# MobilePerceptionLab/EventCalib

Measured on NVIDIA B200. Metric: events/sec (detection+residual eval), higher is better.
Workload: dtype int32 pixels / f64 fit + f64 residuals

## Files before the change

eventcalib_b200/csrc/ecb_api.cu:

```cuda
#include <sched.h>
#include <math.h>
#include <stdarg.h>
#include <stdio.h>
#include <string.h>

#include <algorithm>

#include "ecb_window.cuh"

int ecb_fail(ecb_ctx *ctx, int code, const char *fmt, ...) {
    char buf[512];
    va_list ap;
    va_start(ap, fmt);
    vsnprintf(buf, sizeof buf, fmt, ap);
    va_end(ap);
    if (ctx) ctx->err = buf;
    return code;
}

int ecb_check(ecb_ctx *ctx, cudaError_t e, const char *what) {
    if (e == cudaSuccess) return ECB_OK;
    return ecb_fail(ctx, ECB_ERR_CUDA, "CUDA error %s: %s", what, cudaGetErrorString(e));
}

// ... 282 lines not shown

    if ((rc = ecb_reserve(ctx, ctx->win_t, (size_t) n_win * 16))) return rc;
    if ((rc = ecb_reserve(ctx, ctx->win_lohi, (size_t) n_win * 16))) return rc;
    if ((rc = ecb_reserve(ctx, ctx->win_ptoff, (size_t) n_win * 8))) return rc;
    if ((rc = ecb_h2d(ctx, ctx->win_t.p, windows, (size_t) n_win * 16))) return rc;
    if ((rc = ecb_launch_bounds(ctx, (const double *) ctx->win_t.p, n_win, (int64_t *) ctx->win_lohi.p))) return rc;
    ctx->h_lohi.resize((size_t) 2 * n_win);
    ctx->h_ptoff.resize((size_t) n_win);
    if ((rc = ecb_d2h(ctx, ctx->h_lohi.data(), ctx->win_lohi.p, (size_t) n_win * 16))) return rc;
    int64_t total = 0, max_cnt = 0;
    for (int w = 0; w < n_win; ++w) {
        int64_t cnt = std::max<int64_t>(0, ctx->h_lohi[2 * w + 1] - ctx->h_lohi[2 * w]);
        ctx->h_ptoff[w] = total;
        total += cnt;
        max_cnt = std::max(max_cnt, cnt);
    }
    if (max_cnt > 0x3FFFFFFF) return ecb_fail(ctx, ECB_ERR_UNSUPPORTED, "window with %lld events", (long long) max_cnt);
    ctx->total_points = total;
    if ((rc = ecb_h2d(ctx, ctx->win_ptoff.p, ctx->h_ptoff.data(), (size_t) n_win * 8))) return rc;

    const size_t slots = (size_t) std::max<int64_t>(total, 1);
    if ((rc = ecb_reserve(ctx, ctx->arrive, 2 * slots * 4))) return rc;
    for (int p = 0; p < 2; ++p) {
        if ((rc = ecb_reserve(ctx, ctx->pts[p], slots * 4))) return rc;
        if ((rc = ecb_reserve(ctx, ctx->labels[p], slots * 4))) return rc;
    }
    if ((rc = ecb_reserve(ctx, ctx->kmem, 2 * slots * 4))) return rc;
    if ((rc = ecb_reserve(ctx, ctx->db_dims, (size_t) 2 * n_win * sizeof(ProbDesc)))) return rc;
    if ((rc = ecb_reserve(ctx, ctx->db_hdr, (size_t) 2 * n_win * sizeof(ProbHdr)))) return rc;
    if ((rc = ecb_reserve(ctx, ctx->summary, (size_t) n_win * sizeof(ecb_window_summary)))) return rc;
    if ((rc = ecb_reserve(ctx, ctx->status, 64))) return rc;

    WindowArgs wa;
    wa.xyp = (const uint32_t *) ctx->ev_xyp.p;
    wa.lohi = (const int64_t *) ctx->win_lohi.p;
    wa.ptoff = (const int64_t *) ctx->win_ptoff.p;
    wa.arrive[0] = (uint32_t *) ctx->arrive.p;
    wa.arrive[1] = (uint32_t *) ctx->arrive.p + slots;
    wa.pts[0] = (uint32_t *) ctx->pts[0].p;
    wa.pts[1] = (uint32_t *) ctx->pts[1].p;
    wa.prob = (ProbDesc *) ctx->db_dims.p;
    wa.n_win = n_win;
    wa.W = ctx->width;
    wa.H = ctx->height;
    wa.max_n = (uint32_t *) ctx->status.p + 4;
    wa.order_mode = params->order_mode;
    ECB_CUDA(ctx, cudaMemsetAsync(ctx->status.p, 0, 64, ctx->stream));
    if ((rc = ecb_launch_window(ctx, wa))) return rc;
    uint32_t max_nm[2] = {0, 0};
    if ((rc = ecb_d2h(ctx, max_nm, wa.max_n, 8))) return rc;
    const uint32_t max_n = max_nm[0];
    if (params->order_mode == 1) {
        OrderArgs oa;
        memset(&oa, 0, sizeof oa);
        oa.prob = (const ProbDesc *) ctx->db_dims.p;
        oa.n_prob = 2 * n_win;
        oa.work_counter = (unsigned *) ctx->status.p;
        for (int p = 0; p < 2; ++p) {
            oa.arrive[p] = wa.arrive[p];
            oa.pts[p] = wa.pts[p];
        }
        if ((rc = ecb_launch_order(ctx, oa, (int) max_nm[1]))) return rc;
    }

  for (int attempt = 0;; ++attempt) {
    if ((rc = ecb_reserve(ctx, ctx->ktab, (size_t) 2 * n_win * max_k * sizeof(KeptCluster)))) return rc;
    ctx->cand_stride = max_k;
    if ((rc = ecb_reserve(ctx, ctx->cand, (size_t) n_win * ctx->cand_stride * 5 * 8))) return rc;
    uint32_t *const d_max_kept = (uint32_t *) ctx->status.p + 12;
    ca.max_kept = d_max_kept;
    ca.prob = (const ProbDesc *) ctx->db_dims.p;
    ca.n_prob = 2 * n_win;
    ca.work_counter = (unsigned *) ctx->status.p;
    for (int p = 0; p < 2; ++p) {
        ca.pix[p] = (const uint32_t *) ctx->pts[p].p;
        ca.labels[p] = (int32_t *) ctx->labels[p].p;
        ca.kmem[p] = (uint32_t *) ctx->kmem.p + p * slots;
    }
    ca.hdr = (ProbHdr *) ctx->db_hdr.p;
    ca.ktab = (KeptCluster *) ctx->ktab.p;
    ca.max_k = max_k;
    ca.W = ctx->width;
    ca.H = ctx->height;
    ca.PW = ((ca.W + 2 * ca.E + 31) >> 5) + 1;
    ca.PH = ca.H + 2 * ca.E;
    ca.min_pts = params->dbscan_min_pts;
    ca.cluster_min = params->cluster_min;
    const bool exact = params->median_mode == 1;
    int bfs_cap = 0;
    if (exact) {
        bfs_cap = (int) std::min<size_t>((size_t) 2 * n_win * max_k, 2 * slots / std::max<uint32_t>(params->cluster_min, 1u) + 16);
        if ((rc = ecb_reserve(ctx, ctx->kd_tree, 8 * slots * 4))) return rc;
        if ((rc = ecb_reserve(ctx, ctx->bfs_key, 2 * slots * 8))) return rc;
        if ((rc = ecb_reserve(ctx, ctx->bfs_items, (size_t) bfs_cap * sizeof(BfsItem) + 16))) return rc;
        ca.exact_order = 1;
        for (int p = 0; p < 2; ++p) ca.kd_nodes[p] = (uint32_t *) ctx->kd_tree.p + (size_t) (4 * p) * slots;
        ca.bfs_items = (BfsItem *) ((char *) ctx->bfs_items.p + 16);
        ca.bfs_count = (unsigned *) ctx->bfs_items.p;
        ca.bfs_cap = bfs_cap;
        ECB_CUDA(ctx, cudaMemsetAsync(ctx->bfs_items.p, 0, 16, ctx->stream));
    }
    if ((rc = ecb_launch_cluster(ctx, ca, (int) max_n))) return rc;
    if (exact) {
        BfsArgs ba;
        memset(&ba, 0, sizeof ba);
        ba.items = ca.bfs_items;
        ba.count = ca.bfs_count;
        ba.max_items = bfs_cap;
        ba.prob = ca.prob;
        for (int p = 0; p < 2; ++p) {
            ba.pix[p] = ca.pix[p];
            ba.labels[p] = ca.labels[p];
            ba.kd_nodes[p] = (const uint4 *) ca.kd_nodes[p];
            ba.members[p] = ca.kmem[p];
            ba.scratch[p] = wa.arrive[p];
            ba.key[p] = (unsigned long long *) ctx->bfs_key.p + (size_t) p * slots;
        }
        ba.init_keys = 1;
        ba.ktab = ca.ktab;
        ba.max_k = max_k;
        ba.eps = params->dbscan_eps;
        if ((rc = ecb_launch_bfs(ctx, ba))) return rc;
    }

    PairArgs pa;
    pa.prob = ca.prob;
    pa.hdr = ca.hdr;
    pa.ktab = ca.ktab;
    for (int p = 0; p < 2; ++p) {
        pa.pts[p] = ca.pix[p];
        pa.kmem[p] = ca.kmem[p];
    }
    pa.lohi = wa.lohi;
    pa.summary = (ecb_window_summary *) ctx->summary.p;
    pa.cand = (double *) ctx->cand.p;
    pa.n_win = n_win;
    pa.max_k = max_k;
    pa.cand_stride = ctx->cand_stride;
    pa.smem_cap = (int) max_n;
    pa.fit_circle = params->fit_circle;
    pa.knn_num = params->knn_num < 1 ? 1 : params->knn_num;
    pa.rows_cols = params->rows_cols;
    pa.rthr = params->radius_threshold;
    {
        static const int pair_dyn = getenv("ECB_PAIR_DYN") ? atoi(getenv("ECB_PAIR_DYN")) : 1;
        pa.win_counter = pair_dyn ? (unsigned *) ctx->status.p + 8 : nullptr;
    }
    if ((rc = ecb_launch_pair(ctx, pa))) return rc;
    if (!auto_k) break;
    uint32_t max_kept = 0;
    if ((rc = ecb_d2h(ctx, &max_kept, d_max_kept, 4))) return rc;
    if (max_kept <= (uint32_t) max_k) break;
    if (attempt >= 2) return ecb_fail(ctx, ECB_ERR_STATE, "kept-cluster table still too small after resizing (%u > %d)", max_kept, max_k);
    max_k = (int) ((max_kept + 63u) & ~63u);
    ctx->max_k_auto = max_k;
    ECB_CUDA(ctx, cudaMemsetAsync((uint32_t *) ctx->status.p + 8, 0, 32, ctx->stream));
  }
    ctx->n_win = n_win;
    return ECB_OK;
}

int ecb_frontend_summary(ecb_ctx *ctx, ecb_window_summary *out, int n_win) {
    if (!ctx || !out) return ECB_ERR_ARG;
    if (n_win > ctx->n_win) n_win = ctx->n_win;
    cudaSetDevice(ctx->device);
    return ecb_d2h(ctx, out, ctx->summary.p, (size_t) n_win * sizeof(ecb_window_summary));
}
// ... 122 lines not shown
}

int ecb_frontend_device_ptrs(ecb_ctx *ctx, void **d_summary, void **d_candidates, int *cand_stride) {
    if (!ctx) return ECB_ERR_ARG;
    if (d_summary) *d_summary = ctx->summary.p;
    if (d_candidates) *d_candidates = ctx->cand.p;
    if (cand_stride) *cand_stride = ctx->cand_stride;
    return ECB_OK;
}

static int dbscan_batch(ecb_ctx *ctx, const double *xy, const int64_t *offsets, int n_problems, double eps,
                        uint32_t min_pts, int32_t *labels, int32_t *n_clusters, uint32_t *status, int32_t *cluster_sizes,
                        uint32_t *members) {
    if (!ctx || !offsets || n_problems < 0 || (!xy && n_problems > 0)) return ECB_ERR_ARG;
    const bool ordered = cluster_sizes && members;
    if (min_pts < 1) return ecb_fail(ctx, ECB_FAILED, "min < 1 (dbscan.h:123)");
    cudaSetDevice(ctx->device);
    int rc;
    ClusterArgs ca;
    memset(&ca, 0, sizeof ca);
    if (n_problems == 0) return ECB_OK;
    auto general = [&]() {
        if (status)
            for (int k = 0; k < n_problems; ++k) status[k] = 0;
        return ecb_dbscan_general(ctx, xy, 2, offsets, n_problems, eps, min_pts, labels, n_clusters, cluster_sizes, members);
    };
    if (!(eps >= 1.0) || eps > ECB_MAX_EPS) return general();
    if ((rc = fill_stencil(ctx, ca, eps))) return rc;
    const int64_t total = offsets[n_problems];
    std::vector<uint32_t> pix((size_t) std::max<int64_t>(total, 1));
    std::vector<ProbDesc> pd((size_t) n_problems);
    int Wmax = 1, Hmax = 1, max_n = 0;
    for (int k = 0; k < n_problems; ++k) {
        const int64_t b = offsets[k], e = offsets[k + 1];
        if (e - b < 1) return ecb_fail(ctx, ECB_FAILED, "problem %d: V->size() < 1 (dbscan.h:121)", k);
        if (e - b > 0x3FFFFFFF) return ecb_fail(ctx, ECB_ERR_UNSUPPORTED, "problem %d too large", k);
        int xmin = 1 << 30, ymin = 1 << 30, xmax = -1, ymax = -1;
        for (int64_t i = b; i < e; ++i) {
            const double x = xy[2 * i], y = xy[2 * i + 1];
            const int xi = (int) x, yi = (int) y;
            if (!(x >= 0.0 && x < 32768.0 && y >= 0.0 && y < 32768.0 && (double) xi == x && (double) yi == y)) return general();
            pix[(size_t) i] = (uint32_t) xi | ((uint32_t) yi << 15);
            xmin = std::min(xmin, xi);
            ymin = std::min(ymin, yi);
            xmax = std::max(xmax, xi);
            ymax = std::max(ymax, yi);
        }
        ProbDesc d;
        memset(&d, 0, sizeof d);
        d.off = b;
        d.n = (int32_t) (e - b);
        d.pol = 0;
        d.x0 = xmin;
        d.y0 = ymin;
        pd[(size_t) k] = d;
        Wmax = std::max(Wmax, xmax - xmin + 1);
        Hmax = std::max(Hmax, ymax - ymin + 1);
        max_n = std::max(max_n, d.n);
    }
    if ((int64_t) (Wmax + 2 * ca.E + 64) * (Hmax + 2 * ca.E) > (1ll << 21)) return general();
    const size_t slots = (size_t) std::max<int64_t>(total, 1);
    const int max_k = 1;
    if ((rc = ecb_reserve(ctx, ctx->db_pix, slots * 4))) return rc;
    if ((rc = ecb_reserve(ctx, ctx->db_labels, slots * 4))) return rc;
    if ((rc = ecb_reserve(ctx, ctx->db_scratch, slots * 4))) return rc;
    if ((rc = ecb_reserve(ctx, ctx->db_off, (size_t) n_problems * sizeof(ProbDesc)))) return rc;
    if ((rc = ecb_reserve(ctx, ctx->db_hdr_b, (size_t) n_problems * sizeof(ProbHdr)))) return rc;
    if ((rc = ecb_reserve(ctx, ctx->db_ktab, (size_t) n_problems * max_k * sizeof(KeptCluster)))) return rc;
    if ((rc = ecb_reserve(ctx, ctx->db_counter, 64))) return rc;
    ECB_CUDA(ctx, cudaMemcpyAsync(ctx->db_pix.p, pix.data(), slots * 4, cudaMemcpyHostToDevice, ctx->stream));
    ECB_CUDA(ctx, cudaMemcpyAsync(ctx->db_off.p, pd.data(), (size_t) n_problems * sizeof(ProbDesc), cudaMemcpyHostToDevice,
                                  ctx->stream));
    ca.prob = (const ProbDesc *) ctx->db_off.p;
    ca.n_prob = n_problems;
    ca.work_counter = (unsigned *) ctx->db_counter.p;
    ca.pix[0] = ca.pix[1] = (const uint32_t *) ctx->db_pix.p;
    ca.labels[0] = ca.labels[1] = (int32_t *) ctx->db_labels.p;
    ca.kmem[0] = ca.kmem[1] = (uint32_t *) ctx->db_scratch.p;
    ca.hdr = (ProbHdr *) ctx->db_hdr_b.p;
    ca.ktab = (KeptCluster *) ctx->db_ktab.p;
    ca.max_k = max_k;
    ca.W = Wmax;
    ca.H = Hmax;
    ca.PW = ((ca.W + 2 * ca.E + 31) >> 5) + 1;
    ca.PH = ca.H + 2 * ca.E;
    ca.min_pts = min_pts;
    ca.cluster_min = 0x7FFFFFFF;
    ca.max_kept = nullptr;
    if (ordered) {
        if ((rc = ecb_reserve(ctx, ctx->kd_tree, 4 * slots * 4))) return rc;
        ca.exact_order = 1;
        ca.kd_nodes[0] = ca.kd_nodes[1] = (uint32_t *) ctx->kd_tree.p;
        ca.bfs_count = (unsigned *) ctx->db_counter.p + 4;
        ca.bfs_cap = 0;
    }
    if ((rc = ecb_launch_cluster(ctx, ca, max_n))) return rc;
    if (ordered) {
        if ((rc = ecb_reserve(ctx, ctx->bfs_key, slots * 8))) return rc;
        if ((rc = ecb_reserve(ctx, ctx->bfs_items, slots * sizeof(BfsItem) + 16))) return rc;
        if ((rc = ecb_reserve(ctx, ctx->bfs_front, slots * 4))) return rc;
        if ((rc = ecb_reserve(ctx, ctx->bfs_tab, 3 * slots * 4))) return rc;
        ECB_CUDA(ctx, cudaMemsetAsync(ctx->bfs_key.p, 0xFF, slots * 8, ctx->stream));
        ECB_CUDA(ctx, cudaMemsetAsync(ctx->bfs_items.p, 0, 16, ctx->stream));
        uint32_t *csize = (uint32_t *) ctx->bfs_tab.p, *cseed = csize + slots, *coff = cseed + slots;
        BfsItem *items = (BfsItem *) ((char *) ctx->bfs_items.p + 16);
        if ((rc = ecb_launch_bfs_all_items(ctx, ca.prob, ca.hdr, n_problems, ca.labels[0], csize, cseed, coff, items,
                                           (unsigned *) ctx->bfs_items.p, (int) slots)))
            return rc;
        BfsArgs ba;
        memset(&ba, 0, sizeof ba);
        ba.items = items;
        ba.count = (const unsigned *) ctx->bfs_items.p;
        ba.max_items = (int) slots;
        ba.prob = ca.prob;
        for (int p = 0; p < 2; ++p) {
            ba.pix[p] = ca.pix[0];
            ba.labels[p] = ca.labels[0];
            ba.kd_nodes[p] = (const uint4 *) ca.kd_nodes[0];
            ba.members[p] = (uint32_t *) ctx->db_scratch.p;
            ba.scratch[p] = (uint32_t *) ctx->bfs_front.p;
            ba.key[p] = (unsigned long long *) ctx->bfs_key.p;
        }
        ba.init_keys = 0;
        ba.eps = eps;
        if ((rc = ecb_launch_bfs(ctx, ba))) return rc;
        ECB_CUDA(ctx, cudaMemcpyAsync(members, ctx->db_scratch.p, (size_t) total * 4, cudaMemcpyDeviceToHost, ctx->stream));
        ECB_CUDA(ctx, cudaMemcpyAsync(cluster_sizes, csize, (size_t) total * 4, cudaMemcpyDeviceToHost, ctx->stream));
    }
    std::vector<ProbHdr> hdr((size_t) n_problems);
    if (labels) ECB_CUDA(ctx, cudaMemcpyAsync(labels, ctx->db_labels.p, (size_t) total * 4, cudaMemcpyDeviceToHost, ctx->stream));
    ECB_CUDA(ctx, cudaMemcpyAsync(hdr.data(), ctx->db_hdr_b.p, (size_t) n_problems * sizeof(ProbHdr), cudaMemcpyDeviceToHost,
                                  ctx->stream));
    ECB_CUDA(ctx, ecb_stream_sync(ctx));
    for (int k = 0; k < n_problems; ++k) {
        if (n_clusters) n_clusters[k] = hdr[(size_t) k].n_clusters;
        if (status) status[k] = hdr[(size_t) k].status;
        if (hdr[(size_t) k].status & ECB_PB_DUPLICATE) return general();
    }
    return ECB_OK;
}

int ecb_dbscan_run_batch(ecb_ctx *ctx, const double *xy, const int64_t *offsets, int n_problems, double eps,
                         uint32_t min_pts, int32_t *labels, int32_t *n_clusters, uint32_t *status) {
    return dbscan_batch(ctx, xy, offsets, n_problems, eps, min_pts, labels, n_clusters, status, nullptr, nullptr);
}

int ecb_dbscan_run_batch_ordered(ecb_ctx *ctx, const double *xy, const int64_t *offsets, int n_problems, double eps,
                                 uint32_t min_pts, int32_t *labels, int32_t *n_clusters, uint32_t *status,
                                 int32_t *cluster_sizes, uint32_t *members) {
    if (!cluster_sizes || !members) return ECB_ERR_ARG;
    return dbscan_batch(ctx, xy, offsets, n_problems, eps, min_pts, labels, n_clusters, status, cluster_sizes, members);
}

int ecb_dbscan_run_ordered(ecb_ctx *ctx, const double *xy, int n, double eps, uint32_t min_pts, int32_t *labels,
                           int32_t *n_clusters, int32_t *cluster_sizes, uint32_t *members) {
    if (!ctx || !cluster_sizes || !members) return ECB_ERR_ARG;
    if (n < 1 || min_pts < 1) return ECB_FAILED;
    const int64_t off[2] = {0, n};
    return dbscan_batch(ctx, xy, off, 1, eps, min_pts, labels, n_clusters, nullptr, cluster_sizes, members);
}

int ecb_dbscan_run_nd(ecb_ctx *ctx, const double *pts, int n, int dim, double eps, uint32_t min_pts, int32_t *labels,
                      int32_t *n_clusters, int32_t *cluster_sizes, uint32_t *members) {
    if (!ctx || (!pts && n > 0) || ((cluster_sizes == nullptr) != (members == nullptr))) return ECB_ERR_ARG;
    if (n < 1 || dim < 1 || min_pts < 1) return ECB_FAILED;
    const int64_t off[2] = {0, n};
    if (dim == 2) return dbscan_batch(ctx, pts, off, 1, eps, min_pts, labels, n_clusters, nullptr, cluster_sizes, members);
// ... 85 lines not shown
```

eventcalib_b200/csrc/ecb_cluster.cu:

```cuda
#include <stdlib.h>

#include <algorithm>

#include "ecb_cluster.cuh"

namespace {

template <typename RankT>
struct Smem {
    uint32_t *U, *C;
    RankT *wrank;
    uint32_t *r_pix, *r_lab, *r_kd, *r_st;
    uint8_t *r_flag;
};

#ifndef ECB_CL_RANKORDER
#define ECB_CL_RANKORDER 1
#endif
#ifndef ECB_CL_ROLL
#define ECB_CL_ROLL 1
#endif
#ifndef ECB_CL_UNSET
#define ECB_CL_UNSET 1
#endif

constexpr int KD_PT = 6;

__device__ __forceinline__ uint32_t find_root(volatile uint32_t *parent, uint32_t a) {
    uint32_t p = parent[a];
    while (p != a) {
        uint32_t g = parent[p];
        if (g != p) parent[a] = g;
        a = p;
        p = g;
    }
    return a;
}

__device__ __forceinline__ void unite(uint32_t *parent, uint32_t a, uint32_t b) {
    for (;;) {
        a = find_root(parent, a);
        b = find_root(parent, b);
        if (a == b) return;
        if (a < b) {
            uint32_t t = a;
            a = b;
            b = t;
        }
        if (atomicCAS(&parent[a], a, b) == a) return;
    }
}

template <typename RankT, bool SM>
__global__ void __launch_bounds__(ECB_CL_THREADS, 2) k_cluster(const ClusterArgs a) {
    extern __shared__ __align__(16) uint32_t smem_raw[];
    __shared__ uint32_t ws[33];
    __shared__ uint32_t s_nextpb[2], s_status, s_chunk;
    __shared__ uint8_t s_own[ECB_CL_THREADS / 32][32];

    const int tid = threadIdx.x, nthr = blockDim.x, lane = tid & 31, wid = tid >> 5, nwarp = nthr >> 5;
    const int PW = a.PW, PH = a.PH, E = a.E, NW = PW * PH;
    Smem<RankT> s;
    const int plane_words = 2 * NW + (int) ((NW * sizeof(RankT) + 3) / 4);
    uint32_t *arr;
    if constexpr (SM) {
        s.U = smem_raw;
        arr = smem_raw + plane_words;
    } else {
        uint32_t *gs = a.gscratch + (size_t) blockIdx.x * a.gscratch_stride;
        s.U = a.planes_in_smem ? smem_raw : gs;
        arr = a.planes_in_smem ? gs : gs + plane_words;
    }
    s.C = s.U + NW;
    s.wrank = reinterpret_cast<RankT *>(s.C + NW);
    const int NC = a.n_cap;
    s.r_pix = arr;
    s.r_lab = arr + NC;
    s.r_kd = arr + 2 * NC;
    s.r_st = arr + 4 * NC;
    s.r_flag = reinterpret_cast<uint8_t *>(arr + 5 * NC);
    int32_t *k_raw = reinterpret_cast<int32_t *>(arr + 5 * NC + ((NC + 3) >> 2));
    int32_t *k_size = k_raw + a.max_k, *k_off = k_size + a.max_k;

    for (int i = tid; i < 2 * NW; i += nthr) s.U[i] = 0;
    if (tid == 0) {
        s_nextpb[0] = atomicAdd(a.work_counter, 1u);
        s_status = 0;
    }
    for (int iter = 0;; ++iter) {
#if !ECB_CL_UNSET
        __syncthreads();
        for (int i = tid; i < 2 * NW; i += nthr) s.U[i] = 0;
#endif
        __syncthreads();
        const uint32_t pb = s_nextpb[iter & 1];
        if (pb >= (uint32_t) a.n_prob) break;
        uint32_t next_pb = 0;
        if (tid == 0) next_pb = atomicAdd(a.work_counter, 1u);
        const ProbDesc d = a.prob[pb];
        const int n = d.n;
        const uint32_t *gpix = a.pix[d.pol] + d.off;
        int32_t *glab = a.labels[d.pol] + d.off;
        for (int pid = tid; pid < n; pid += nthr) {
            uint32_t p = gpix[pid];
            int x = (int) ECB_PIX_X(p) - d.x0, y = (int) ECB_PIX_Y(p) - d.y0;
            uint32_t loc = ECB_NONE;
            if (x >= 0 && x < a.W && y >= 0 && y < a.H && !(p & ECB_PIX_INVALID)) {
                x += E;
                y += E;
                uint32_t bit = 1u << (x & 31);
                uint32_t old = atomicOr(&s.U[y * PW + (x >> 5)], bit);
                if (old & bit)
                    atomicOr(&s_status, ECB_PB_DUPLICATE);
                else
                    loc = (uint32_t) x | ((uint32_t) y << 16);
            } else {
                atomicOr(&s_status, ECB_PB_RANGE);
            }
            s.r_pix[pid] = loc;
        }
        __syncthreads();
        uint32_t n_ranked;
        {
            const int per = (NW + nthr - 1) / nthr;
            const int b = tid * per, e = min(NW, b + per);
            uint32_t c = 0;
#if ECB_CL_ROLL
#pragma unroll 1
#endif
            for (int i = b; i < e; ++i) c += __popc(s.U[i]);
            uint32_t ex = block_excl_scan(c, ws, &n_ranked);
#if ECB_CL_ROLL
#pragma unroll 1
#endif
            for (int i = b; i < e; ++i) {
                s.wrank[i] = (RankT) ex;
                ex += __popc(s.U[i]);
            }
        }
        __syncthreads();
        auto rank_of = [&](int x, int y) -> uint32_t {
            const int w = y * PW + (x >> 5);
            return (uint32_t) s.wrank[w] + __popc(s.U[w] & ((1u << (x & 31)) - 1u));
        };
        uint32_t *child = s.r_kd;
        uint32_t *rloc = s.r_lab;
        for (int i = tid; i < 2 * n; i += nthr) child[i] = ECB_NONE;
        if (n <= KD_PT * nthr) {
            uint32_t mypix[KD_PT], cur[KD_PT], fl[KD_PT];
#pragma unroll
            for (int k = 0; k < KD_PT; ++k) {
                const int pid = tid + k * nthr;
                mypix[k] = pid < n ? s.r_pix[pid] : ECB_NONE;
                cur[k] = (pid == 0 || mypix[k] == ECB_NONE) ? ECB_NONE : 0u;
                fl[k] = 0;
            }
            __syncthreads();
            for (int round = 0;; ++round) {
                const int dsh = (round & 1) ? 16 : 0;
                bool any = false;
                uint32_t slot[KD_PT];
#pragma unroll
                for (int k = 0; k < KD_PT; ++k) {
                    if (cur[k] == ECB_NONE) continue;
                    any = true;
                    const uint32_t ci = (mypix[k] >> dsh) & 0xFFFF, ca = (s.r_pix[cur[k]] >> dsh) & 0xFFFF;
                    if (ci == ca) fl[k] |= 1u << (round & 1);
                    slot[k] = 2 * cur[k] + (ci < ca ? 0 : 1);
                    atomicMin(&child[slot[k]], (uint32_t) (tid + k * nthr));
                }
                if (!__syncthreads_or(any)) break;
#pragma unroll
                for (int k = 0; k < KD_PT; ++k) {
                    if (cur[k] == ECB_NONE) continue;
                    const uint32_t c = child[slot[k]];
                    cur[k] = c == (uint32_t) (tid + k * nthr) ? ECB_NONE : c;
                }
            }
#pragma unroll
            for (int k = 0; k < KD_PT; ++k)
                if (mypix[k] != ECB_NONE) {
                    const uint32_t rk = rank_of(mypix[k] & 0xFFFF, mypix[k] >> 16);
                    s.r_flag[rk] = (uint8_t) fl[k];
                    rloc[rk] = mypix[k];
                    s.r_st[tid + k * nthr] = rk;
                }
        } else {
            uint32_t *state = s.r_st;
            const uint32_t DONE = 0x3FFFFFFFu;
            for (int pid = tid; pid < n; pid += nthr) state[pid] = (pid == 0 || s.r_pix[pid] == ECB_NONE) ? DONE : 0u;
            __syncthreads();
            for (int round = 0;; ++round) {
                const int dsh = (round & 1) ? 16 : 0;
                bool any = false;
                for (int pid = tid; pid < n; pid += nthr) {
                    uint32_t st = state[pid];
                    uint32_t cur = st & DONE;
                    if (cur == DONE) continue;
                    any = true;
                    uint32_t ci = (s.r_pix[pid] >> dsh) & 0xFFFF, ca = (s.r_pix[cur] >> dsh) & 0xFFFF;
                    if (ci == ca) state[pid] = st | (0x40000000u << (round & 1));
                    atomicMin(&child[2 * cur + (ci < ca ? 0 : 1)], (uint32_t) pid);
                }
                if (!__syncthreads_or(any)) break;
                for (int pid = tid; pid < n; pid += nthr) {
                    uint32_t st = state[pid];
                    uint32_t cur = st & DONE;
                    if (cur == DONE) continue;
                    uint32_t ci = (s.r_pix[pid] >> dsh) & 0xFFFF, ca = (s.r_pix[cur] >> dsh) & 0xFFFF;
                    uint32_t c = child[2 * cur + (ci < ca ? 0 : 1)];
                    state[pid] = (st & 0xC0000000u) | (c == (uint32_t) pid ? DONE : c);
                }
                __syncthreads();
            }
            for (int pid = tid; pid < n; pid += nthr) {
                const uint32_t loc = s.r_pix[pid];
                if (loc != ECB_NONE) {
                    const uint32_t rk = rank_of(loc & 0xFFFF, loc >> 16);
                    s.r_flag[rk] = (uint8_t) (state[pid] >> 30);
                    rloc[rk] = loc;
                    state[pid] = rk;
                }
            }
        }
        __syncthreads();
        if (a.exact_order) {
            uint32_t *nodes = a.kd_nodes[d.pol] + 4 * d.off;
            for (int pid = tid; pid < n; pid += nthr) {
                const uint32_t l = child[2 * pid], r = child[2 * pid + 1];
                nodes[4 * pid] = gpix[pid];
                nodes[4 * pid + 1] = l;
                nodes[4 * pid + 2] = r;
                if (l != ECB_NONE) nodes[4 * l + 3] = (uint32_t) pid;
                if (r != ECB_NONE) nodes[4 * r + 3] = (uint32_t) pid;
            }
            if (tid == 0 && n > 0) nodes[3] = ECB_NONE;
            __syncthreads();
        }
        auto flag_of = [&](int x, int y) -> uint32_t { return s.r_flag[rank_of(x, y)]; };
        const int ei = a.eps_int;
        const int m = (int) n_ranked;
        for (int it5 = tid; it5 < (ECB_CL_RANKORDER ? m : n); it5 += nthr) {
            int rk = it5;
            if (!ECB_CL_RANKORDER) {
                if (s.r_pix[it5] == ECB_NONE) continue;
                rk = (int) s.r_st[it5];
            }
            const uint32_t loc = rloc[rk];
            const int x = loc & 0xFFFF, y = loc >> 16;
            int cnt = -1;
            for (int dy = -E; dy <= E; ++dy) {
                const int w = a.halfw[dy < 0 ? -dy : dy];
                cnt += __popc(row_bits(s.U + (y + dy) * PW, x - w, 2 * w + 1));
            }
            if (ei > 0) {
                if (test_bit(s.U + y * PW, x + ei)) cnt -= (int) (flag_of(x + ei, y) & 1u);
                if (test_bit(s.U + (y + ei) * PW, x)) cnt -= (int) ((flag_of(x, y + ei) >> 1) & 1u);
            }
            if (cnt >= (int) a.min_pts) atomicOr(&s.C[y * PW + (x >> 5)], 1u << (x & 31));
        }
        uint32_t *parent = s.r_kd, *glabel = s.r_kd + NC;
        for (int r = tid; r < n; r += nthr) {
            parent[r] = r;
            glabel[r] = ECB_NONE;
        }
        __syncthreads();
        const int gap = (ei > 0 ? ei : E + 1) - 1;
        for (int it6 = tid; it6 < (ECB_CL_RANKORDER ? m : n); it6 += nthr) {
            int rk = it6;
            if (!ECB_CL_RANKORDER) {
// ... 68 lines not shown
                for (int it0 = 0; it0 < n_it; it0 += 32) {
                    const int it = it0 + lane;
                    const bool act = it < n_it;
                    const int hi = act ? (int) (((uint32_t) it * invE) >> 16) : 0;
                    const int dy = it - hi * E + 1;
                    const int owner = (int) s_own[wid][hi];
                    const uint32_t loc = __shfl_sync(0xffffffffu, h_xy, owner);
                    const uint32_t sub = __shfl_sync(0xffffffffu, h_sub, owner);
                    const uint32_t rf = __shfl_sync(0xffffffffu, h_rf, owner);
                    if (!act) continue;
                    const int x = loc & 0xFFFF, y = loc >> 16, j = x >> 5;
                    const int w = a.halfw[dy];
                    const uint32_t *tr = s.C + (y + dy) * PW + j;
                    const uint32_t T0 = j > 0 ? tr[-1] : 0u, T1 = tr[0], T2 = j + 1 < PW ? tr[1] : 0u;
                    if (!(T0 | T1 | T2)) continue;
                    const uint64_t Tw = ((uint64_t) T0 >> 16) | ((uint64_t) T1 << 16) | ((uint64_t) T2 << 48);
                    uint64_t d64 = ((uint64_t) sub << 16) >> w;
                    for (int k = 0; k < 2 * w;) {
                        const int add = min(k + 1, 2 * w - k);
                        d64 |= d64 << add;
                        k += add;
                    }
                    uint64_t hits = d64 & Tw;
                    if (!hits) continue;
                    if (dy != ei) hits &= ~smear(hits);
                    while (hits) {
                        const int nx = 32 * j - 16 + (__ffsll((long long) hits) - 1);
                        hits &= hits - 1;
                        if (dy == ei && (flag_of(nx, y + dy) & 2u)) continue;
                        unite(parent, rf, rank_of(nx, y + dy));
                    }
                }
                __syncwarp();
            }
        }
        __syncthreads();
        int n_core_local = 0;
        for (int pid = tid; pid < n; pid += nthr) {
            uint32_t loc = s.r_pix[pid];
            uint32_t root = ECB_NONE;
            if (loc != ECB_NONE) {
                const int x = loc & 0xFFFF, y = loc >> 16;
                if (test_bit(s.C + y * PW, x)) {
                    ++n_core_local;
                    root = find_root(parent, s.r_st[pid]);
                    atomicMin(&glabel[root], (uint32_t) pid);
                }
            }
            s.r_lab[pid] = root;
        }
        __syncthreads();
        for (int pid = tid; pid < n; pid += nthr) {
            const uint32_t root = s.r_lab[pid];
            if (root != ECB_NONE) parent[s.r_st[pid]] = root;
        }
        __syncthreads();
        if (ei > 0) {
            for (;;) {
                bool changed = false;
                for (int pid = tid; pid < n; pid += nthr) {
                    const uint32_t gq = s.r_lab[pid];
                    if (gq == ECB_NONE) continue;
                    const uint32_t loc = s.r_pix[pid];
                    const int x = loc & 0xFFFF, y = loc >> 16;
                    if (test_bit(s.C + y * PW, x + ei)) {
                        const uint32_t rp = rank_of(x + ei, y);
                        if (s.r_flag[rp] & 1u) {
                            uint32_t lp = ((volatile uint32_t *) glabel)[parent[rp]];
                            if (lp < atomicMin(&glabel[gq], lp)) changed = true;
                        }
                    }
                    if (test_bit(s.C + (y + ei) * PW, x)) {
                        const uint32_t rp = rank_of(x, y + ei);
                        if (s.r_flag[rp] & 2u) {
                            uint32_t lp = ((volatile uint32_t *) glabel)[parent[rp]];
                            if (lp < atomicMin(&glabel[gq], lp)) changed = true;
                        }
                    }
                }
                if (!__syncthreads_or(changed)) break;
            }
        }
        const int nw32 = (n + 31) >> 5;
        uint32_t *seedmask = s.r_st, *seedpref = s.r_st + nw32;
        for (int i = tid; i < nw32; i += nthr) seedmask[i] = 0;
        __syncthreads();
        for (int pid = tid; pid < n; pid += nthr) {
            const uint32_t g = s.r_lab[pid];
            if (g == ECB_NONE) continue;
            if (glabel[g] == (uint32_t) pid) atomicOr(&seedmask[pid >> 5], 1u << (pid & 31));
        }
        __syncthreads();
        uint32_t n_clusters;
        {
            const int per = (nw32 + nthr - 1) / nthr;
            const int b = tid * per, e = min(nw32, b + per);
            uint32_t c = 0;
#if ECB_CL_ROLL
#pragma unroll 1
#endif
            for (int i = b; i < e; ++i) c += __popc(seedmask[i]);
            uint32_t ex = block_excl_scan(c, ws, &n_clusters);
#if ECB_CL_ROLL
#pragma unroll 1
#endif
            for (int i = b; i < e; ++i) {
                seedpref[i] = ex;
                ex += __popc(seedmask[i]);
            }
        }
        __syncthreads();
        for (int pid = tid; pid < n; pid += nthr) {
            const uint32_t g = s.r_lab[pid];
            int32_t lab = -1;
            if (g != ECB_NONE) {
                const uint32_t seed = glabel[g];
                lab = (int32_t) (seedpref[seed >> 5] + __popc(seedmask[seed >> 5] & ((1u << (seed & 31)) - 1u)));
            }
            s.r_lab[pid] = (uint32_t) lab;
            glab[pid] = lab;
            const uint32_t loc = s.r_pix[pid];
            if (ECB_CL_UNSET && loc != ECB_NONE) {
                const int w = (int) (loc >> 16) * PW + (int) ((loc & 0xFFFF) >> 5);
                s.U[w] = 0;
                s.C[w] = 0;
            }
        }
        __syncthreads();
        const int nc = (int) n_clusters;
        uint32_t *csize = s.r_kd, *keptidx = s.r_kd + nc;
        for (int i = tid; i < nc; i += nthr) csize[i] = 0;
        __syncthreads();
        for (int pid = tid; pid < n; pid += nthr) {
            int32_t lab = (int32_t) s.r_lab[pid];
            if (lab >= 0) atomicAdd(&csize[lab], 1u);
        }
        __syncthreads();
        uint32_t n_kept = 0;
        {
            const int per = (nc + nthr - 1) / nthr;
            const int b = tid * per, e = min(nc, b + per);
            uint32_t c = 0;
#if ECB_CL_ROLL
#pragma unroll 1
#endif
            for (int i = b; i < e; ++i) c += csize[i] >= a.cluster_min;
            uint32_t ex = block_excl_scan(c, ws, &n_kept);
#if ECB_CL_ROLL
#pragma unroll 1
#endif
            for (int i = b; i < e; ++i) {
                const bool k = csize[i] >= a.cluster_min;
                keptidx[i] = k ? ex : ECB_NONE;
                if (k && ex < (uint32_t) a.max_k) {
                    k_raw[ex] = i;
                    k_size[ex] = (int32_t) csize[i];
                }
                ex += k;
            }
        }
        if (n_kept > (uint32_t) a.max_k) {
            if (tid == 0) {
                atomicOr(&s_status, ECB_PB_CLUSTER_CAP);
                if (a.max_kept) atomicMax(a.max_kept, n_kept);
            }
            n_kept = a.max_k;
        }
        __syncthreads();
        if (wid == 0) {
            uint32_t run = 0;
#if ECB_CL_ROLL
#pragma unroll 1
#endif
            for (int base = 0; base < (int) n_kept; base += 32) {
                uint32_t v = base + lane < (int) n_kept ? (uint32_t) k_size[base + lane] : 0;
                uint32_t inc = warp_incl_scan(v);
                if (base + lane < (int) n_kept) k_off[base + lane] = (int32_t) (run + inc - v);
                run += __shfl_sync(0xffffffffu, inc, 31);
            }
            if (lane == 0) k_off[n_kept] = (int32_t) run;
        }
        __syncthreads();
        uint32_t *members = s.r_st;
        uint32_t *gmem = a.kmem[d.pol] + d.off;
        KeptCluster *kt = a.ktab + (size_t) pb * a.max_k;
        if (n_kept > 0) {
            const int L = (((n + nwarp - 1) / nwarp) + 31) & ~31;
            const int p0 = wid * L, p1 = min(n, p0 + L);
            auto kept_of = [&](int pid) -> int {
                if (pid >= p1) return -1;
                const int32_t lab = (int32_t) s.r_lab[pid];
                if (lab < 0) return -1;
                const uint32_t ki = keptidx[lab];
                return (ki != ECB_NONE && ki < n_kept) ? (int) ki : -1;
            };
            if ((int) n_kept * nwarp <= 2 * NC - 2 * nc) {
                uint32_t *cnt = s.r_kd + 2 * nc;
                for (int i = tid; i < (int) n_kept * nwarp; i += nthr) cnt[i] = 0;
                __syncthreads();
                uint32_t *mycnt = cnt + wid * n_kept;
                for (int c = p0; c < p1; c += 32) {
                    const int kidx = kept_of(c + lane);
                    const uint32_t peers = __match_any_sync(0xffffffffu, kidx);
                    if (kidx >= 0 && (peers & ((1u << lane) - 1u)) == 0) mycnt[kidx] += __popc(peers);
                    __syncwarp();
                }
                __syncthreads();
#if ECB_CL_ROLL
#pragma unroll 1
#endif
                for (int k = tid; k < (int) n_kept; k += nthr) {
                    uint32_t run = 0;
#if ECB_CL_ROLL
#pragma unroll 1
#endif
                    for (int w = 0; w < nwarp; ++w) {
                        const uint32_t t = cnt[w * n_kept + k];
                        cnt[w * n_kept + k] = run;
                        run += t;
                    }
                }
                __syncthreads();
                for (int c = p0; c < p1; c += 32) {
                    const int pid = c + lane;
                    const int kidx = kept_of(pid);
                    const uint32_t peers = __match_any_sync(0xffffffffu, kidx);
                    const int rk = __popc(peers & ((1u << lane) - 1u));
                    uint32_t base = 0;
                    if (kidx >= 0) {
                        base = mycnt[kidx];
                        members[k_off[kidx] + base + rk] = pid;
                    }
                    __syncwarp();
                    if (kidx >= 0 && rk == 0) mycnt[kidx] = base + __popc(peers);
                    __syncwarp();
                }
            } else {
                for (int k = wid; k < (int) n_kept; k += nwarp) {
                    const int32_t cid = k_raw[k];
                    const int base = k_off[k];
                    int pos = 0;
                    for (int st = 0; st < n; st += 32) {
                        const int pid = st + lane;
                        const bool m = pid < n && (int32_t) s.r_lab[pid] == cid;
                        const uint32_t ball = __ballot_sync(0xffffffffu, m);
                        if (m) members[base + pos + __popc(ball & ((1u << lane) - 1u))] = pid;
                        pos += __popc(ball);
                    }
                }
            }
        }
        __syncthreads();
        const int pbits = 32 - __clz(max(n - 1, 1));
        const unsigned long long maxn2 = (unsigned long long) (a.W - 1 + d.x0) * (a.W - 1 + d.x0) +
                                         (unsigned long long) (a.H - 1 + d.y0) * (a.H - 1 + d.y0);
        const bool key32 = pbits < 32 && maxn2 < (1ull << (32 - pbits));
        for (int k = wid; k < (int) n_kept; k += nwarp) {
            const int32_t cid = k_raw[k];
            const int base = k_off[k], sz = k_size[k];
            unsigned long long S[9] = {0, 0, 0, 0, 0, 0, 0, 0, 0};
            int med = -1;
            uint32_t *mnorm = s.r_kd;
            for (int i = lane; i < sz; i += 32) {
                const uint32_t pid = members[base + i];
                gmem[base + i] = pid;
                const uint32_t loc = s.r_pix[pid];
                const uint32_t x = (uint32_t) ((int) (loc & 0xFFFF) - E + d.x0), y = (uint32_t) ((int) (loc >> 16) - E + d.y0);
                const uint32_t xx = x * x, yy = y * y, xy = x * y;
                S[0] += x;
                S[1] += y;
                S[2] += xx;
                S[3] += yy;
                S[4] += xy;
                S[5] += (unsigned long long) xx * x;
                S[6] += (unsigned long long) yy * y;
                S[7] += (unsigned long long) xy * y;
                S[8] += (unsigned long long) xx * y;
                mnorm[base + i] = xx + yy;
            }
            __syncwarp();
            bool tie = false;
            if (key32) {
#if ECB_CL_ROLL
#pragma unroll 1
#endif
                for (int i = lane; i < sz; i += 32) mnorm[base + i] = (mnorm[base + i] << pbits) | members[base + i];
                __syncwarp();
                uint32_t mkey = 0;
                for (int i = lane; i < sz; i += 32) {
                    const uint32_t ki = mnorm[base + i];
                    int cnt = 0;
                    for (int j = 0; j < sz; ++j) cnt += mnorm[base + j] < ki;
                    if (cnt == sz / 2) mkey = ki;
                }
#pragma unroll
                for (int o = 16; o > 0; o >>= 1) mkey = max(mkey, __shfl_xor_sync(0xffffffffu, mkey, o));
                med = (int) (mkey & ((1u << pbits) - 1u));
                int eq = 0;
#if ECB_CL_ROLL
#pragma unroll 1
#endif
                for (int i = lane; i < sz; i += 32) eq += (mnorm[base + i] >> pbits) == (mkey >> pbits);
                tie = __reduce_add_sync(0xffffffffu, eq) > 1;
                if (lane != 0) med = -1;
            } else {
                for (int i = lane; i < sz; i += 32) {
                    const uint32_t ni = mnorm[base + i], pi = members[base + i];
                    int cnt = 0, eq = 0;
                    for (int j = 0; j < sz; ++j) {
                        const uint32_t nj = mnorm[base + j], pj = members[base + j];
                        cnt += (nj < ni) || (nj == ni && pj < pi);
                        eq += nj == ni;
                    }
                    if (cnt == sz / 2) {
                        med = (int) pi;
                        tie = eq > 1;
                    }
                }
            }
            if (a.exact_order && __any_sync(0xffffffffu, tie) && lane == 0) {
                const unsigned slot = atomicAdd(a.bfs_count, 1u);
                if (slot < (unsigned) a.bfs_cap) {
                    BfsItem it;
                    it.pb = (int32_t) pb;
                    it.cid = cid;
                    it.seed = (int32_t) members[base];
                    it.size = sz;
                    it.mem_off = base;
                    it.kept = k;
                    a.bfs_items[slot] = it;
                }
            }
#pragma unroll
            for (int q = 0; q < 9; ++q) {
                const uint32_t l0 = __reduce_add_sync(0xffffffffu, (uint32_t) S[q] & 0x1FFFFFu);
                const uint32_t l1 = __reduce_add_sync(0xffffffffu, (uint32_t) (S[q] >> 21) & 0x1FFFFFu);
                const uint32_t l2 = __reduce_add_sync(0xffffffffu, (uint32_t) (S[q] >> 42));
                S[q] = (unsigned long long) l0 + ((unsigned long long) l1 << 21) + ((unsigned long long) l2 << 42);
            }
            med = __reduce_max_sync(0xffffffffu, med);
            if (lane == 0) {
                KeptCluster kc;
                kc.raw_id = cid;
                kc.size = sz;
                kc.med_pid = med;
                const uint32_t lm = s.r_pix[med];
                kc.med_x = (int) (lm & 0xFFFF) - E + d.x0;
                kc.med_y = (int) (lm >> 16) - E + d.y0;
                kc.mem_off = base;
#pragma unroll
                for (int q = 0; q < 9; ++q) kc.m[q] = (double) S[q];
                kt[k] = kc;
            }
        }
        {
            uint32_t tot;
            block_excl_scan((uint32_t) n_core_local, ws, &tot);
            if (tid == 0) {
                ProbHdr h;
                h.n_clusters = nc;
                h.n_kept = (int32_t) n_kept;
                h.n_core = (int32_t) tot;
                h.status = s_status;
                a.hdr[pb] = h;
                s_status = 0;
                s_nextpb[(iter + 1) & 1] = next_pb;
            }
        }
    }
}

}

static size_t cluster_array_words(int n_cap, int max_k) { return (size_t) 5 * n_cap + ((size_t) n_cap + 3) / 4 + (size_t) 3 * max_k + 1; }

size_t ecb_cluster_smem_bytes(int PW, int PH, int n_cap, int max_k, bool arrays_in_smem, bool rank32) {
    size_t NW = (size_t) PW * PH;
    size_t b = 2 * NW * 4 + ((NW * (rank32 ? 4 : 2) + 3) / 4) * 4;
    if (arrays_in_smem) b += cluster_array_words(n_cap, max_k) * 4;
    return b;
}

int ecb_launch_cluster(ecb_ctx *ctx, ClusterArgs &a, int max_n) {
    if (a.n_prob <= 0) return ECB_OK;
    const bool rank32 = max_n >= 65535;
    a.n_cap = max_n < 64 ? 64 : max_n;
    const size_t limit = (size_t) ctx->smem_optin - 9 * 1024;
    size_t planes = ecb_cluster_smem_bytes(a.PW, a.PH, a.n_cap, a.max_k, false, rank32);
    size_t with_arrays = ecb_cluster_smem_bytes(a.PW, a.PH, a.n_cap, a.max_k, true, rank32);
    a.planes_in_smem = planes <= limit;
    a.arrays_in_smem = with_arrays <= limit;
    size_t smem = a.arrays_in_smem ? with_arrays : (a.planes_in_smem ? planes : 0);
    int per_sm = 1;
    void (*kern)(const ClusterArgs) = rank32 ? (a.arrays_in_smem ? k_cluster<uint32_t, true> : k_cluster<uint32_t, false>)
                                             : (a.arrays_in_smem ? k_cluster<uint16_t, true> : k_cluster<uint16_t, false>);
    ECB_CUDA(ctx, cudaFuncSetAttribute(kern, cudaFuncAttributeMaxDynamicSharedMemorySize, (int) limit));
    int by_smem = 1;
    ECB_CUDA(ctx, cudaOccupancyMaxActiveBlocksPerMultiprocessor(&by_smem, kern, 32, smem));
    int threads = std::max(128, std::min(ECB_CL_THREADS, (1024 / std::max(by_smem, 1)) & ~31));
    if (!a.arrays_in_smem) threads = ECB_CL_THREADS;
    if (const char *e = getenv("ECB_CL_THREADS")) threads = std::max(64, std::min(ECB_CL_THREADS, atoi(e) & ~31));
    ECB_CUDA(ctx, cudaOccupancyMaxActiveBlocksPerMultiprocessor(&per_sm, kern, threads, smem));
    if (per_sm < 1) per_sm = 1;
    int grid = ctx->sm_count * per_sm;
    if (grid > a.n_prob) grid = a.n_prob;
    if (!a.arrays_in_smem) {
        a.gscratch_stride = cluster_array_words(a.n_cap, a.max_k) + (a.planes_in_smem ? 0 : (planes + 3) / 4);
        int rc = ecb_reserve(ctx, ctx->scratch, (size_t) grid * a.gscratch_stride * 4);
        if (rc) return rc;
        a.gscratch = (uint32_t *) ctx->scratch.p;
    }
    ECB_CUDA(ctx, cudaMemsetAsync(a.work_counter, 0, 4, ctx->stream));
    ECB_PROF_BEGIN(ctx, ECB_STAGE_CLUSTER);
    kern<<<grid, threads, smem, ctx->stream>>>(a);
    ECB_PROF_END(ctx, ECB_STAGE_CLUSTER);
    ECB_LAUNCHED(ctx);
    return ecb_check(ctx, cudaGetLastError(), "k_cluster launch");
}
```

eventcalib_b200/csrc/ecb_cluster.cuh:

```cuda
#pragma once
#include "ecb_common.cuh"

#define ECB_CL_THREADS 512

struct ProbDesc {
    int64_t off;
    int32_t n;
    int32_t pol;
    int32_t x0, y0;
    int32_t pad0, pad1;
};

struct ProbHdr {
    int32_t n_clusters;
    int32_t n_kept;
    int32_t n_core;
    uint32_t status;
};

struct KeptCluster {
    int32_t raw_id;
    int32_t size;
    int32_t med_pid;
    int32_t med_x, med_y;
    int32_t mem_off;
    double m[9];
};

struct BfsItem {
    int32_t pb;
    int32_t cid;
    int32_t seed;
    int32_t size;
    int32_t mem_off;
    int32_t kept;
};

struct ClusterArgs {
    const ProbDesc *prob;
    int n_prob;
    unsigned *work_counter;
    const uint32_t *pix[2];
    int32_t *labels[2];
    uint32_t *kmem[2];
    ProbHdr *hdr;
    KeptCluster *ktab;
    int max_k;
    uint32_t *max_kept;
    uint32_t *gscratch;
    size_t gscratch_stride;
    int arrays_in_smem;
    int planes_in_smem;
    int n_cap;
    int W, H, E, PW, PH;
    int eps_int;
    uint32_t min_pts, cluster_min;
    int8_t halfw[ECB_MAX_EPS + 1];
    int exact_order;
    uint32_t *kd_nodes[2];
    BfsItem *bfs_items;
    unsigned *bfs_count;
    int bfs_cap;
};

struct BfsArgs {
    const BfsItem *items;
    const unsigned *count;
    int max_items;
    const ProbDesc *prob;
    const uint32_t *pix[2];
    const int32_t *labels[2];
    const uint4 *kd_nodes[2];
    uint32_t *members[2];
    uint32_t *scratch[2];
    unsigned long long *key[2];
    int init_keys;
    KeptCluster *ktab;
    int max_k;
    double eps;
};

size_t ecb_cluster_smem_bytes(int PW, int PH, int n_cap, int max_k, bool arrays_in_smem, bool rank32);
int ecb_launch_cluster(ecb_ctx *ctx, ClusterArgs &a, int max_n);
int ecb_launch_bfs(ecb_ctx *ctx, BfsArgs &a);
int ecb_launch_bfs_general(ecb_ctx *ctx, BfsArgs &a, const double *P, int dim);
int ecb_sort_events_by_time(ecb_ctx *ctx, int64_t n);
int ecb_dbscan_general(ecb_ctx *ctx, const double *pts, int dim, const int64_t *offsets, int n_problems, double eps,
                       uint32_t min_pts, int32_t *labels, int32_t *n_clusters, int32_t *cluster_sizes, uint32_t *members);
int ecb_launch_bfs_all_items(ecb_ctx *ctx, const ProbDesc *prob, const ProbHdr *hdr, int n_prob, const int32_t *labels,
                             uint32_t *csize, uint32_t *cseed, uint32_t *coff, BfsItem *items, unsigned *count, int cap);
```

Baseline: 2.522 billion.

## Use 64-bit rank words, drop row padding word, and add 16-bit state arrays

The occupancy-bitmap rank table now holds one entry per pair of 32-bit words and uses 64-bit popcounts. This halves the rank array and the prefix-scan work. The per-row padding word is dropped, which shrinks the bitmap planes. A new kernel variant stores the state/member array as uint16 when n_cap < 32768 so more problem data fits in shared memory. The launcher picks the variant in a loop. Risks: the rank_of change alters how bits near row edges are handled once the padding word is removed, the 64-bit reads need 8-byte-aligned plane bases, and the state path for 16-bit StT appears only partly implemented (the else branch is now restricted to 4-byte StT).

New measurement: 2.618 billion (median of 6 runs). +3.8%, better.

```diff
diff --git a/eventcalib_b200/csrc/ecb_api.cu b/eventcalib_b200/csrc/ecb_api.cu
--- a/eventcalib_b200/csrc/ecb_api.cu
+++ b/eventcalib_b200/csrc/ecb_api.cu
@@ -388,7 +388,7 @@
     ca.max_k = max_k;
     ca.W = ctx->width;
     ca.H = ctx->height;
-    ca.PW = ((ca.W + 2 * ca.E + 31) >> 5) + 1;
+    ca.PW = ecb_cluster_row_words(ca.W, ca.E);
     ca.PH = ca.H + 2 * ca.E;
     ca.min_pts = params->dbscan_min_pts;
     ca.cluster_min = params->cluster_min;
@@ -677,7 +677,7 @@
     ca.max_k = max_k;
     ca.W = Wmax;
     ca.H = Hmax;
-    ca.PW = ((ca.W + 2 * ca.E + 31) >> 5) + 1;
+    ca.PW = ecb_cluster_row_words(ca.W, ca.E);
     ca.PH = ca.H + 2 * ca.E;
     ca.min_pts = min_pts;
     ca.cluster_min = 0x7FFFFFFF;
diff --git a/eventcalib_b200/csrc/ecb_cluster.cu b/eventcalib_b200/csrc/ecb_cluster.cu
--- a/eventcalib_b200/csrc/ecb_cluster.cu
+++ b/eventcalib_b200/csrc/ecb_cluster.cu
@@ -6,11 +6,12 @@
 
 namespace {
 
-template <typename RankT>
+template <typename RankT, typename StT>
 struct Smem {
     uint32_t *U, *C;
     RankT *wrank;
-    uint32_t *r_pix, *r_lab, *r_kd, *r_st;
+    uint32_t *r_pix, *r_lab, *r_kd;
+    StT *r_st;
     uint8_t *r_flag;
 };
 
@@ -51,7 +52,7 @@
     }
 }
 
-template <typename RankT, bool SM>
+template <typename RankT, typename StT, bool SM>
 __global__ void __launch_bounds__(ECB_CL_THREADS, 2) k_cluster(const ClusterArgs a) {
     extern __shared__ __align__(16) uint32_t smem_raw[];
     __shared__ uint32_t ws[33];
@@ -60,8 +61,9 @@
 
     const int tid = threadIdx.x, nthr = blockDim.x, lane = tid & 31, wid = tid >> 5, nwarp = nthr >> 5;
     const int PW = a.PW, PH = a.PH, E = a.E, NW = PW * PH;
-    Smem<RankT> s;
-    const int plane_words = 2 * NW + (int) ((NW * sizeof(RankT) + 3) / 4);
+    const int NP = (NW + 1) >> 1;
+    Smem<RankT, StT> s;
+    const int plane_words = 2 * NW + (int) ((NP * sizeof(RankT) + 3) / 4);
     uint32_t *arr;
     if constexpr (SM) {
         s.U = smem_raw;
@@ -77,9 +79,10 @@
     s.r_pix = arr;
     s.r_lab = arr + NC;
     s.r_kd = arr + 2 * NC;
-    s.r_st = arr + 4 * NC;
-    s.r_flag = reinterpret_cast<uint8_t *>(arr + 5 * NC);
-    int32_t *k_raw = reinterpret_cast<int32_t *>(arr + 5 * NC + ((NC + 3) >> 2));
+    const int st_words = sizeof(StT) == 4 ? NC : (NC + 1) >> 1;
+    s.r_st = reinterpret_cast<StT *>(arr + 4 * NC);
+    s.r_flag = reinterpret_cast<uint8_t *>(arr + (4 * NC + st_words));
+    int32_t *k_raw = reinterpret_cast<int32_t *>(arr + (4 * NC + st_words + ((NC + 3) >> 2)));
     int32_t *k_size = k_raw + a.max_k, *k_off = k_size + a.max_k;
 
     for (int i = tid; i < 2 * NW; i += nthr) s.U[i] = 0;
@@ -120,28 +123,30 @@
             s.r_pix[pid] = loc;
         }
         __syncthreads();
+        auto pair_bits = [&](int i) -> uint64_t { return 2 * i + 1 < NW ? reinterpret_cast<const uint64_t *>(s.U)[i] : (uint64_t) s.U[2 * i]; };
         uint32_t n_ranked;
         {
-            const int per = (NW + nthr - 1) / nthr;
-            const int b = tid * per, e = min(NW, b + per);
+            const int per = (NP + nthr - 1) / nthr;
+            const int b = tid * per, e = min(NP, b + per);
             uint32_t c = 0;
 #if ECB_CL_ROLL
 #pragma unroll 1
 #endif
-            for (int i = b; i < e; ++i) c += __popc(s.U[i]);
+            for (int i = b; i < e; ++i) c += __popcll(pair_bits(i));
             uint32_t ex = block_excl_scan(c, ws, &n_ranked);
 #if ECB_CL_ROLL
 #pragma unroll 1
 #endif
             for (int i = b; i < e; ++i) {
                 s.wrank[i] = (RankT) ex;
-                ex += __popc(s.U[i]);
+                ex += __popcll(pair_bits(i));
             }
         }
         __syncthreads();
         auto rank_of = [&](int x, int y) -> uint32_t {
             const int w = y * PW + (x >> 5);
-            return (uint32_t) s.wrank[w] + __popc(s.U[w] & ((1u << (x & 31)) - 1u));
+            const int b = ((w & 1) << 5) | (x & 31);
+            return (uint32_t) s.wrank[w >> 1] + __popcll(reinterpret_cast<const uint64_t *>(s.U)[w >> 1] & ((1ull << b) - 1ull));
         };
         uint32_t *child = s.r_kd;
         uint32_t *rloc = s.r_lab;
@@ -183,9 +188,9 @@
                     const uint32_t rk = rank_of(mypix[k] & 0xFFFF, mypix[k] >> 16);
                     s.r_flag[rk] = (uint8_t) fl[k];
                     rloc[rk] = mypix[k];
-                    s.r_st[tid + k * nthr] = rk;
-                }
-        } else {
+                    s.r_st[tid + k * nthr] = (StT) rk;
+                }
+        } else if constexpr (sizeof(StT) == 4) {
             uint32_t *state = s.r_st;
             const uint32_t DONE = 0x3FFFFFFFu;
             for (int pid = tid; pid < n; pid += nthr) state[pid] = (pid == 0 || s.r_pix[pid] == ECB_NONE) ? DONE : 0u;
@@ -420,7 +425,7 @@
             }
         }
         const int nw32 = (n + 31) >> 5;
-        uint32_t *seedmask = s.r_st, *seedpref = s.r_st + nw32;
+        uint32_t *seedmask = reinterpret_cast<uint32_t *>(s.r_st), *seedpref = seedmask + nw32;
         for (int i = tid; i < nw32; i += nthr) seedmask[i] = 0;
         __syncthreads();
         for (int pid = tid; pid < n; pid += nthr) {
@@ -519,7 +524,7 @@
             if (lane == 0) k_off[n_kept] = (int32_t) run;
         }
         __syncthreads();
-        uint32_t *members = s.r_st;
+        StT *members = s.r_st;
         uint32_t *gmem = a.kmem[d.pol] + d.off;
         KeptCluster *kt = a.ktab + (size_t) pb * a.max_k;
         if (n_kept > 0) {
@@ -567,7 +572,7 @@
                     uint32_t base = 0;
                     if (kidx >= 0) {
                         base = mycnt[kidx];
-                        members[k_off[kidx] + base + rk] = pid;
+                        members[k_off[kidx] + base + rk] = (StT) pid;
                     }
                     __syncwarp();
                     if (kidx >= 0 && rk == 0) mycnt[kidx] = base + __popc(peers);
@@ -582,7 +587,7 @@
                         const int pid = st + lane;
                         const bool m = pid < n && (int32_t) s.r_lab[pid] == cid;
                         const uint32_t ball = __ballot_sync(0xffffffffu, m);
-                        if (m) members[base + pos + __popc(ball & ((1u << lane) - 1u))] = pid;
+                        if (m) members[base + pos + __popc(ball & ((1u << lane) - 1u))] = (StT) pid;
                         pos += __popc(ball);
                     }
                 }
@@ -710,12 +715,15 @@
 
 }
 
-static size_t cluster_array_words(int n_cap, int max_k) { return (size_t) 5 * n_cap + ((size_t) n_cap + 3) / 4 + (size_t) 3 * max_k + 1; }
-
-size_t ecb_cluster_smem_bytes(int PW, int PH, int n_cap, int max_k, bool arrays_in_smem, bool rank32) {
-    size_t NW = (size_t) PW * PH;
-    size_t b = 2 * NW * 4 + ((NW * (rank32 ? 4 : 2) + 3) / 4) * 4;
-    if (arrays_in_smem) b += cluster_array_words(n_cap, max_k) * 4;
+static size_t cluster_array_words(int n_cap, int max_k, bool st16) {
+    return (size_t) 4 * n_cap + (st16 ? ((size_t) n_cap + 1) / 2 : (size_t) n_cap) + ((size_t) n_cap + 3) / 4 +
+           (size_t) 3 * max_k + 1;
+}
+
+size_t ecb_cluster_smem_bytes(int PW, int PH, int n_cap, int max_k, bool arrays_in_smem, bool rank32, bool st16) {
+    size_t NP = ((size_t) PW * PH + 1) / 2;
+    size_t b = (size_t) PW * PH * 8 + ((NP * (rank32 ? 4 : 2) + 3) / 4) * 4;
+    if (arrays_in_smem) b += cluster_array_words(n_cap, max_k, st16) * 4;
     return b;
 }
 
@@ -724,26 +732,34 @@
     const bool rank32 = max_n >= 65535;
     a.n_cap = max_n < 64 ? 64 : max_n;
     const size_t limit = (size_t) ctx->smem_optin - 9 * 1024;
-    size_t planes = ecb_cluster_smem_bytes(a.PW, a.PH, a.n_cap, a.max_k, false, rank32);
-    size_t with_arrays = ecb_cluster_smem_bytes(a.PW, a.PH, a.n_cap, a.max_k, true, rank32);
+    const size_t planes = ecb_cluster_smem_bytes(a.PW, a.PH, a.n_cap, a.max_k, false, rank32, false);
     a.planes_in_smem = planes <= limit;
-    a.arrays_in_smem = with_arrays <= limit;
-    size_t smem = a.arrays_in_smem ? with_arrays : (a.planes_in_smem ? planes : 0);
+    void (*kern)(const ClusterArgs) = nullptr;
+    size_t smem = 0;
+    int threads = ECB_CL_THREADS;
+    for (int st16 = a.n_cap < 32768; st16 >= 0; --st16) {
+        const size_t with_arrays = ecb_cluster_smem_bytes(a.PW, a.PH, a.n_cap, a.max_k, true, rank32, st16);
+        a.arrays_in_smem = with_arrays <= limit;
+        if (st16 && !a.arrays_in_smem) continue;
+        smem = a.arrays_in_smem ? with_arrays : (a.planes_in_smem ? planes : 0);
+        kern = st16 ? k_cluster<uint16_t, uint16_t, true>
+             : rank32 ? (a.arrays_in_smem ? k_cluster<uint32_t, uint32_t, true> : k_cluster<uint32_t, uint32_t, false>)
+                      : (a.arrays_in_smem ? k_cluster<uint16_t, uint32_t, true> : k_cluster<uint16_t, uint32_t, false>);
+        ECB_CUDA(ctx, cudaFuncSetAttribute(kern, cudaFuncAttributeMaxDynamicSharedMemorySize, (int) limit));
+        int by_smem = 1;
+        ECB_CUDA(ctx, cudaOccupancyMaxActiveBlocksPerMultiprocessor(&by_smem, kern, 32, smem));
+        threads = std::max(128, std::min(ECB_CL_THREADS, (1024 / std::max(by_smem, 1)) & ~31));
+        if (!a.arrays_in_smem) threads = ECB_CL_THREADS;
+        if (const char *e = getenv("ECB_CL_THREADS")) threads = std::max(64, std::min(ECB_CL_THREADS, atoi(e) & ~31));
+        if (!st16 || a.n_cap <= KD_PT * threads) break;
+    }
     int per_sm = 1;
-    void (*kern)(const ClusterArgs) = rank32 ? (a.arrays_in_smem ? k_cluster<uint32_t, true> : k_cluster<uint32_t, false>)
-                                             : (a.arrays_in_smem ? k_cluster<uint16_t, true> : k_cluster<uint16_t, false>);
-    ECB_CUDA(ctx, cudaFuncSetAttribute(kern, cudaFuncAttributeMaxDynamicSharedMemorySize, (int) limit));
-    int by_smem = 1;
-    ECB_CUDA(ctx, cudaOccupancyMaxActiveBlocksPerMultiprocessor(&by_smem, kern, 32, smem));
-    int threads = std::max(128, std::min(ECB_CL_THREADS, (1024 / std::max(by_smem, 1)) & ~31));
-    if (!a.arrays_in_smem) threads = ECB_CL_THREADS;
-    if (const char *e = getenv("ECB_CL_THREADS")) threads = std::max(64, std::min(ECB_CL_THREADS, atoi(e) & ~31));
     ECB_CUDA(ctx, cudaOccupancyMaxActiveBlocksPerMultiprocessor(&per_sm, kern, threads, smem));
     if (per_sm < 1) per_sm = 1;
     int grid = ctx->sm_count * per_sm;
     if (grid > a.n_prob) grid = a.n_prob;
     if (!a.arrays_in_smem) {
-        a.gscratch_stride = cluster_array_words(a.n_cap, a.max_k) + (a.planes_in_smem ? 0 : (planes + 3) / 4);
+        a.gscratch_stride = (cluster_array_words(a.n_cap, a.max_k, false) + (a.planes_in_smem ? 0 : (planes + 3) / 4) + 1) & ~(size_t) 1;
         int rc = ecb_reserve(ctx, ctx->scratch, (size_t) grid * a.gscratch_stride * 4);
         if (rc) return rc;
         a.gscratch = (uint32_t *) ctx->scratch.p;
diff --git a/eventcalib_b200/csrc/ecb_cluster.cuh b/eventcalib_b200/csrc/ecb_cluster.cuh
--- a/eventcalib_b200/csrc/ecb_cluster.cuh
+++ b/eventcalib_b200/csrc/ecb_cluster.cuh
@@ -80,7 +80,8 @@
     double eps;
 };
 
-size_t ecb_cluster_smem_bytes(int PW, int PH, int n_cap, int max_k, bool arrays_in_smem, bool rank32);
+size_t ecb_cluster_smem_bytes(int PW, int PH, int n_cap, int max_k, bool arrays_in_smem, bool rank32, bool st16);
+static inline int ecb_cluster_row_words(int W, int E) { return (W + 2 * E + 31) >> 5; }
 int ecb_launch_cluster(ecb_ctx *ctx, ClusterArgs &a, int max_n);
 int ecb_launch_bfs(ecb_ctx *ctx, BfsArgs &a);
 int ecb_launch_bfs_general(ecb_ctx *ctx, BfsArgs &a, const double *P, int dim);
```
